# amolahinge/739-839-federated-learning-using-grpc

Measured on AMD Instinct MI355X. Metric: rounds/sec + samples/sec/client, 2-conv CNN FedAvg at 1/2/4/8 MI355X clients, higher is better.
Workload: dtype bf16; 1 GPU; model=lenet, global_batch=128, parallelism=fedavg-dp1, per_client_batch=128, local_epochs_per_round=1, eval_per_round=True, eval_split=full-per-client, data_split=strided-iid, aggregation=none (single client), hip_graph=True

## Files before the change

csrc/kernels/lenet_kernels.hip:

```cpp
#include <stdexcept>

#include "common.h"
#include "lenet_layout.h"

using namespace lenet;

#ifdef FEDMI_STAMPS
__device__ unsigned long long fedmi_stamps[FEDMI_STAMP_KERNELS][FEDMI_STAMP_WGS][FEDMI_STAMP_SLOTS];
__device__ int fedmi_ks1_diag;
#endif

namespace {

constexpr int NT_FWD = 512;
constexpr int NW_FWD = NT_FWD / 64;
constexpr int NT_CONV = 1024;
constexpr int NW_CONV = NT_CONV / 64;
constexpr int NT_FC = 512;

__constant__ float kMean[3] = {0.4914f, 0.4822f, 0.4465f};
__constant__ float kInvStd[3] = {1.f / 0.2023f, 1.f / 0.1994f, 1.f / 0.2010f};

FEDMI_DEV bf16x8 ld8(const bf16* p) { return *reinterpret_cast<const bf16x8*>(p); }

// ... 200 lines not shown
    const bf16* __restrict__ pk, const float* __restrict__ params, float* __restrict__ part)
{
  constexpr int SX_LD = F0P + 8;
  constexpr int XCH = F0P / 8;
  __shared__ __attribute__((aligned(16))) bf16 sX[16 * SX_LD];
  __shared__ __attribute__((aligned(16))) bf16 sH1[16 * 128];
  __shared__ __attribute__((aligned(16))) bf16 sH2[16 * 96];
  __shared__ float sZ[16 * 16];
  const int tid = threadIdx.x, lane = lane_id(), wave = wave_id();
  const int kq = (lane >> 4) * 8, n16 = lane & 15, rq = (lane >> 4) * 4;
  const int mt = blockIdx.x, s0 = mt * FC_SPW;
  const int ns = min(FC_SPW, nb - s0);
  if (ns <= 0) return;

  const int nf1 = wave * 16 + n16;
  bf16x8 w1f[13];
#pragma unroll
  for (int ks = 0; ks < 13; ++ks) w1f[ks] = ld8(pk + PK_FC1 + nf1 * F0P + ks * 32 + kq);
  const float b1 = params[P_F1B + min(nf1, F1 - 1)];
  const int nf2 = (wave < 6 ? wave : 0) * 16 + n16;
  const float b2 = params[P_F2B + min(nf2, F2 - 1)];
  const float b3 = params[P_F3B + min(n16, NCLS - 1)];
  bf16x8 w2f[4], w3f[3];
  if (wave < 6) {
#pragma unroll
    for (int ks = 0; ks < 4; ++ks) w2f[ks] = ld8(pk + PK_FC2 + nf2 * 128 + ks * 32 + kq);
  }
  if (wave == 0) {
#pragma unroll
    for (int ks = 0; ks < 3; ++ks) w3f[ks] = ld8(pk + PK_FC3 + n16 * 96 + ks * 32 + kq);
  }
  uint4 xv[2] = {make_uint4(0, 0, 0, 0), make_uint4(0, 0, 0, 0)};
#pragma unroll
  for (int u = 0; u < 2; ++u) {
    const int e = tid + u * NT_FC;
    if (e < 16 * XCH) {
      const int r = e / XCH;
      xv[u] = reinterpret_cast<const uint4*>(act2 + (size_t)(s0 + min(r, ns - 1)) * F0P)[e - r * XCH];
      if (r >= ns) xv[u] = make_uint4(0, 0, 0, 0);
    }
  }
#pragma unroll
  for (int u = 0; u < 2; ++u) {
    const int e = tid + u * NT_FC;
    if (e < 16 * XCH) {
      const int r = e / XCH;
      *reinterpret_cast<uint4*>(sX + r * SX_LD + (e - r * XCH) * 8) = xv[u];
    }
  }
  __syncthreads();

  {
    const bf16* xa = sX + n16 * SX_LD + kq;
    f32x4 acc = zero4();
#pragma unroll
    for (int ks = 0; ks < 13; ++ks) acc = mfma16(ld8(xa + ks * 32), w1f[ks], acc);
#pragma unroll
    for (int r = 0; r < 4; ++r) {
      const int sr = rq + r;
      sH1[sr * 128 + nf1] = (bf16)((nf1 < F1 && sr < ns) ? fmaxf(acc[r] + b1, 0.f) : 0.f);
    }
  }
  __syncthreads();
  if (wave < 6) {
    const bf16* ha = sH1 + n16 * 128 + kq;
    f32x4 acc = zero4();
#pragma unroll
    for (int ks = 0; ks < 4; ++ks) acc = mfma16(ld8(ha + ks * 32), w2f[ks], acc);
#pragma unroll
    for (int r = 0; r < 4; ++r) {
      const int sr = rq + r;
      sH2[sr * 96 + nf2] = (bf16)((nf2 < F2 && sr < ns) ? fmaxf(acc[r] + b2, 0.f) : 0.f);
    }
  }
  __syncthreads();
  if (wave == 0) {
    const bf16* ha = sH2 + n16 * 96 + kq;
    f32x4 acc = zero4();
#pragma unroll
    for (int ks = 0; ks < 3; ++ks) acc = mfma16(ld8(ha + ks * 32), w3f[ks], acc);
#pragma unroll
    for (int r = 0; r < 4; ++r) sZ[(rq + r) * 16 + n16] = acc[r] + b3;
  }
  __syncthreads();
  if (wave == 0) {
    float loss = 0.f, corr = 0.f;
    if (lane < ns) {
      float z[NCLS];
#pragma unroll
      for (int n = 0; n < NCLS; ++n) z[n] = sZ[lane * 16 + n];
      float mx = z[0]; int am = 0;
#pragma unroll
      for (int n = 1; n < NCLS; ++n) if (z[n] > mx) { mx = z[n]; am = n; }
      float se = 0.f;
#pragma unroll
      for (int n = 0; n < NCLS; ++n) se += __expf(z[n] - mx);
      const int y = labels[s0 + lane];
      float zy = 0.f;
#pragma unroll
      for (int n = 0; n < NCLS; ++n) zy = (n == y) ? z[n] : zy;
      loss = mx + __logf(se) - zy;
      corr = (am == y) ? 1.f : 0.f;
    }
    loss = wave_sum(loss);
    corr = wave_sum(corr);
    if (lane == 0) {
      part[2 * mt] = loss;
      part[2 * mt + 1] = corr;
    }
  }
}

constexpr int BW_XROW = 40, BW_XS_C = 32 * BW_XROW + 72, BW_XS_S = 3 * BW_XS_C + 48;
constexpr int BW_XSH = 5 * BW_XS_S;
constexpr int BW_P1SH = 5 * 6 * 14 * 16;
constexpr int BW_DY2W = 16 * 160;
constexpr int BW_DY2S = 24;
constexpr int BW_DY2C = 18 * 18 * BW_DY2S;
constexpr int BW_DY1S = 904;
constexpr int BW_DY1 = 6 * BW_DY1S;
constexpr int BW_WDGS = KDGP + 8;
constexpr int BW_O_XSH = 0, BW_O_P1SH = BW_O_XSH + BW_XSH * 2, BW_O_DY2W = BW_O_P1SH + BW_P1SH * 2,
              BW_O_DY2C = BW_O_DY2W + BW_DY2W * 2, BW_O_DY1 = BW_O_DY2C + BW_DY2C * 2,
              BW_O_DW1 = BW_O_DY1 + BW_DY1 * 2, BW_O_DB = BW_O_DW1 + 3 * 6 * 80 * 4, BW_SCRATCH = BW_O_DB + 64 * 4;

struct BwdLds {
  const uint8_t* raw;
  const bf16* p1r;
  const uint8_t* am1s;
  const uint8_t* am2s;
  const float* dxs;
  const bf16* wdg;
  bf16* xsh; bf16* p1sh; bf16* dY2w; bf16* dY2c; bf16* dY1; float* db; float* w1part;
};

FEDMI_DEV BwdLds bwd_lds(unsigned char* scratch, const uint8_t* raw, const bf16* p1r, const uint8_t* am1s,
                         const uint8_t* am2s, const float* dxs, const bf16* wdg) {
  BwdLds L;
  L.raw = raw; L.p1r = p1r; L.am1s = am1s; L.am2s = am2s; L.dxs = dxs; L.wdg = wdg;
  L.xsh = reinterpret_cast<bf16*>(scratch + BW_O_XSH);
  L.p1sh = reinterpret_cast<bf16*>(scratch + BW_O_P1SH);
  L.dY2w = reinterpret_cast<bf16*>(scratch + BW_O_DY2W);
  L.dY2c = reinterpret_cast<bf16*>(scratch + BW_O_DY2C);
  L.dY1 = reinterpret_cast<bf16*>(scratch + BW_O_DY1);
  L.w1part = reinterpret_cast<float*>(scratch + BW_O_DW1);
  L.db = reinterpret_cast<float*>(scratch + BW_O_DB);
  return L;
}

FEDMI_DEV void bwd_zero(const BwdLds& L) {
  zero_lds<NT_CONV>(L.dY2w, BW_DY2W * 2);
  zero_lds<NT_CONV>(L.dY2c, BW_DY2C * 2);
  zero_lds<NT_CONV>(L.dY1, BW_DY1 * 2);
  zero_lds<NT_CONV>(L.xsh, BW_XSH * 2);
  zero_lds<NT_CONV>(L.p1sh, BW_P1SH * 2);
  if (threadIdx.x < 64) L.db[threadIdx.x] = 0.f;
}

FEDMI_DEV void bwd_build_shifted_img(const BwdLds& L, const Aug& a, int tid, int nthr) {
  for (int e = tid; e < IMG_BYTES; e += nthr) {
    const int c = e >> 10, y = (e >> 5) & 31, x = e & 31;
    const bf16 v = (bf16)aug_pixel(L.raw, a, c, y, x);
    bf16* row = L.xsh + c * BW_XS_C + y * BW_XROW + x;
#pragma unroll
    for (int sh = 0; sh < 5; ++sh)
      if (x >= sh) row[sh * BW_XS_S - sh] = v;
  }
}
FEDMI_DEV void bwd_build_shifted_p1(const BwdLds& L, int tid, int nthr) {
  for (int e = tid; e < NP1; e += nthr) {
    const int c = e / 196, rem = e - c * 196, y = rem / P1, x = rem - y * P1;
    const bf16 v = L.p1r[e];
    bf16* row = L.p1sh + (c * 14 + y) * 16 + x;
#pragma unroll
    for (int sh = 0; sh < 5; ++sh)
      if (x >= sh) row[sh * (6 * 14 * 16) - sh] = v;
  }
}

FEDMI_DEV void bwd_main(const BwdLds& L, float* __restrict__ slab, int sk, int stamp_wg) {
  (void)sk; (void)stamp_wg;
  const int tid = threadIdx.x, lane = lane_id(), wave = wave_id();
  const int kq = (lane >> 4) * 8, n16 = lane & 15, rq = (lane >> 4) * 4;
  float* db = L.db;
  if (tid < C2 * 32) {
    const int o = tid >> 5, rem = tid & 31;
    float g = 0.f;
    if (rem < 25) {
      const int f = o * 25 + rem, py = rem / P2, px = rem - py * P2;
      const int am = L.am2s[f];
      const int y = 2 * py + (am >> 1), x = 2 * px + (am & 1);
      g = L.dxs[f];
      const bf16 gb = (bf16)g;
      L.dY2w[o * 160 + y * 16 + x] = gb;
      L.dY2c[((y + 4) * 18 + (x + 4)) * BW_DY2S + o] = gb;
    }
#pragma unroll
    for (int w = 1; w < 32; w <<= 1) g += __shfl_xor(g, w, 64);
    if (rem == 0) db[o] = g;
  }
  __syncthreads();
  FEDMI_STAMP(sk, 2);

  for (int t = wave - 7; t >= 0 && t < 10; t += 9) {
    const int kk = t * 16 + n16;
    const int kc = kk < 150 ? kk : 0;
    const int c = kc / 25, rs = kc - c * 25, r = rs / 5, sc = rs - r * 5;
    const bf16* bb = L.p1sh + ((sc * 6 + c) * 14 + r) * 16 + (kq & 15);
    f32x4 acc = zero4();
#pragma unroll
    for (int ks = 0; ks < 5; ++ks) {
      const int i = 2 * ks + (kq >> 4);
      acc = mfma16(ld8(L.dY2w + n16 * 160 + ks * 32 + kq), ld8(bb + i * 16), acc);
    }
    if (kk < 150) {
#pragma unroll
      for (int rr = 0; rr < 4; ++rr) slab[P_C2W + (rq + rr) * 150 + kk] = acc[rr];
    }
  }

  int koff[13];
#pragma unroll
  for (int ks = 0; ks < 13; ++ks) {
    const int G = ks * 4 + (lane >> 4), g = G >> 1;
    const int r = g / 5, sc = g - r * 5;
    koff[ks] = g < 25 ? (-r * 18 - sc) * BW_DY2S + (G & 1) * 8 : 0;
  }
  if (wave < 7) {
    const int ta = 2 * wave, tb = 2 * wave + 1;
    int pa = ta * 16 + n16, pb = tb * 16 + n16;
    if (pa >= 196) pa = 0;
    if (pb >= 196) pb = 0;
    const bf16* ga = L.dY2c + (((pa / P1) + 4) * 18 + (pa % P1 + 4)) * BW_DY2S;
    const bf16* gbb = L.dY2c + (((pb / P1) + 4) * 18 + (pb % P1 + 4)) * BW_DY2S;
    const bf16* wb = L.wdg + min(n16, C1) * BW_WDGS + kq;
    f32x4 acc[2] = {zero4(), zero4()};
#pragma unroll
    for (int ks = 0; ks < 13; ++ks) {
      const bf16x8 w = ld8(wb + ks * 32);
      acc[0] = mfma16(ld8(ga + koff[ks]), w, acc[0]);
      acc[1] = mfma16(ld8(gbb + koff[ks]), w, acc[1]);
    }
    FEDMI_STAMP(sk, 6);
    float csum = 0.f;
    if (n16 < C1) {
      const int c = n16;
#pragma unroll
      for (int h = 0; h < 2; ++h) {
        const int t = h ? tb : ta;
#pragma unroll
        for (int rr = 0; rr < 4; ++rr) {
          const int p = t * 16 + rq + rr;
          if (p < 196) {
            const int py = p / P1, px = p - py * P1;
            const float pooled = (float)L.p1r[c * 196 + p];
            const float g = pooled > 0.f ? acc[h][rr] : 0.f;
            const int am = L.am1s[c * 196 + p];
            const int yy = 2 * py + (am >> 1), xx = 2 * px + (am & 1);
            L.dY1[c * BW_DY1S + yy * 32 + xx] = (bf16)g;
            csum += g;
          }
        }
      }
    }
    csum += __shfl_xor(csum, 16, 64);
    csum += __shfl_xor(csum, 32, 64);
    if (n16 < C1 && lane < 16) db[16 + wave * C1 + n16] = csum;
    FEDMI_STAMP(sk, 7);
  }
  __syncthreads();
  FEDMI_STAMP(sk, 3);

  if (wave < 15) {
    const int nt = wave % 5, part = wave / 5;
    const int ks0 = part * 10, ks1 = min(ks0 + 10, O1);
    const int kk = nt * 16 + n16;
    const int kc = kk < 75 ? kk : kk - 64;
    const int c = kc / 25, rs = kc - c * 25, r = rs / 5, sc = rs - r * 5;
    const bf16* bb = L.xsh + sc * BW_XS_S + c * BW_XS_C + r * BW_XROW + kq;
    const bf16* ab = L.dY1 + min(n16, C1 - 1) * BW_DY1S + kq;
    const bool arow = n16 < C1;
    f32x4 acc0 = zero4(), acc1 = zero4();
    int ks = ks0;
    for (; ks + 1 < ks1; ks += 2) {
      bf16x8 a0 = ld8(ab + ks * 32), a1 = ld8(ab + ks * 32 + 32);
      if (!arow) { a0 = zero8(); a1 = zero8(); }
      acc0 = mfma16(a0, ld8(bb + ks * BW_XROW), acc0);
      acc1 = mfma16(a1, ld8(bb + (ks + 1) * BW_XROW), acc1);
    }
    if (ks < ks1) {
      bf16x8 a0 = ld8(ab + ks * 32);
      if (!arow) a0 = zero8();
      acc0 = mfma16(a0, ld8(bb + ks * BW_XROW), acc0);
    }
#pragma unroll
    for (int rr = 0; rr < 4; ++rr) {
      const int o = rq + rr;
      if (o < C1 && kk < 75) L.w1part[(part * 6 + o) * 80 + kk] = acc0[rr] + acc1[rr];
    }
  }
  __syncthreads();
  FEDMI_STAMP(sk, 4);
  for (int e = tid; e < C1 * 75; e += NT_CONV) {
    const int o = e / 75, kk = e - o * 75;
    slab[P_C1W + e] = L.w1part[o * 80 + kk] + L.w1part[(6 + o) * 80 + kk] + L.w1part[(12 + o) * 80 + kk];
  }
  if (tid < C1) {
    float b = 0.f;
#pragma unroll
    for (int w = 0; w < 7; ++w) b += db[16 + w * C1 + tid];
    slab[P_C1B + tid] = b;
  }
  if (tid < C2) slab[P_C2B + tid] = db[tid];
  FEDMI_STAMP(sk, 5);
}

constexpr int AUX_H2T = 0;
constexpr int AUX_DZ2T = AUX_H2T + 96 * 128 * 2;
constexpr int AUX_DZ3T = AUX_DZ2T + 96 * 128 * 2;
constexpr int FCB_N = 224;
constexpr int AUX_FCB = AUX_DZ3T + 16 * 128 * 2;
constexpr int AUX_LOSS = AUX_FCB + MAX_TRAIN_BATCH * FCB_N * 4;
constexpr int AUX_CORR = AUX_LOSS + MAX_TRAIN_BATCH * 4;
constexpr int AUX_BYTES = AUX_CORR + MAX_TRAIN_BATCH * 4;
static_assert(AUX_BYTES <= MAX_TRAIN_BATCH * F0 * 4, "FC side buffers must fit in dact2");

constexpr int S_O_RAW = 0, S_O_P1R = 3072, S_O_AM1 = S_O_P1R + 2368, S_O_AM2 = S_O_AM1 + 1184,
              S_O_X = S_O_AM2 + 416, S_O_DX = S_O_X + F0P * 2, S_O_WDG = S_O_DX + F0 * 4,
              S_O_FC = S_O_WDG + 16 * BW_WDGS * 2, S_O_W1C = S_O_FC + 2048, S_O_W2C = S_O_W1C + 16 * 136 * 2,
              S_O_SCR = S_O_W2C + 16 * 232 * 2;
constexpr int S_W1C_LD = 136, S_W2C_LD = 232;
constexpr int S_F_XCL = 0, S_F_C1 = S_F_XCL + 36 * 40 * 4 * 2, S_F_P1 = S_F_C1 + NPOS1 * 8 * 4,
              S_F_C2 = S_F_P1 + 14 * 14 * 8 * 2, S_F_END = S_F_C2 + C2 * NPOS2 * 4;
constexpr int S_O_RED = S_O_SCR + (S_F_END > BW_SCRATCH ? S_F_END : BW_SCRATCH);
constexpr int S_O_W3 = S_O_RED + NW_CONV * F0P * 4;
constexpr int S_END = S_O_W3 + 16 * 96 * 2;
static_assert(S_END <= 160 * 1024, "KS1 LDS");
constexpr int SF_H1 = 0, SF_H2 = 128, SF_Z = 224, SF_DZ3 = 240, SF_DZ2 = 256, SF_DZ1 = 352, SF_END = 480;
static_assert(SF_END * 4 <= 2048, "FC scratch");

FEDMI_DEV float dot8(const bf16x8& a, const bf16x8& b, float acc) {
#pragma unroll
  for (int j = 0; j < 8; ++j) acc += (float)a[j] * (float)b[j];
  return acc;
}
FEDMI_DEV float dot8f(const float* a, const bf16x8& b, float acc) {
#pragma unroll
  for (int j = 0; j < 8; ++j) acc += a[j] * (float)b[j];
  return acc;
}
FEDMI_DEV float sum8lanes(float v) {
  v += __shfl_xor(v, 1, 64);
  v += __shfl_xor(v, 2, 64);
  v += __shfl_xor(v, 4, 64);
  return v;
}
FEDMI_DEV float bfr(float v) { return (float)(bf16)v; }
FEDMI_DEV float row_sum16(float v) {
  v += __builtin_bit_cast(float, __builtin_amdgcn_mov_dpp(__builtin_bit_cast(int, v), 0x128, 0xf, 0xf, false));
  v += __builtin_bit_cast(float, __builtin_amdgcn_mov_dpp(__builtin_bit_cast(int, v), 0x124, 0xf, 0xf, false));
  v += __builtin_bit_cast(float, __builtin_amdgcn_mov_dpp(__builtin_bit_cast(int, v), 0x122, 0xf, 0xf, false));
  v += __builtin_bit_cast(float, __builtin_amdgcn_mov_dpp(__builtin_bit_cast(int, v), 0x121, 0xf, 0xf, false));
  return v;
}

__global__ __launch_bounds__(NT_CONV) void lenet_sample_step(
    const uint8_t* __restrict__ images, int sample_base, int nb,
    const bf16* __restrict__ pk, const float* __restrict__ params,
    uint32_t seed, const int* __restrict__ round_ctr, int augment,
    const int* __restrict__ labels,
    bf16* __restrict__ act2T,
    bf16* __restrict__ h1T,
    unsigned char* __restrict__ aux,
    bf16* __restrict__ dZ1T,
    float* __restrict__ conv_slab)
{
  __shared__ __attribute__((aligned(16))) unsigned char smem[S_END];
  const int s = blockIdx.x;
  if (s >= nb) return;
  [[maybe_unused]] const int stamp_wg = s;
  const int gidx = sample_base + s;
  const int tid = threadIdx.x, lane = lane_id(), wave = wave_id();
  const int kq = (lane >> 4) * 8, n16 = lane & 15, rq = (lane >> 4) * 4;
  uint8_t* raw = smem + S_O_RAW;
  bf16* p1r = reinterpret_cast<bf16*>(smem + S_O_P1R);
  uint8_t* am1s = smem + S_O_AM1;
  uint8_t* am2s = smem + S_O_AM2;
  bf16* xrow = reinterpret_cast<bf16*>(smem + S_O_X);
  float* dxs = reinterpret_cast<float*>(smem + S_O_DX);
  bf16* wdg = reinterpret_cast<bf16*>(smem + S_O_WDG);
  float* fcs = reinterpret_cast<float*>(smem + S_O_FC);
  float* red = reinterpret_cast<float*>(smem + S_O_RED);
  unsigned char* scr = smem + S_O_SCR;
  bf16* xcl = reinterpret_cast<bf16*>(scr + S_F_XCL);
  float* c1 = reinterpret_cast<float*>(scr + S_F_C1);
  bf16* p1cl = reinterpret_cast<bf16*>(scr + S_F_P1);
  float* c2 = reinterpret_cast<float*>(scr + S_F_C2);
  FEDMI_STAMP(0, 0);

  bf16* w1c = reinterpret_cast<bf16*>(smem + S_O_W1C);
  bf16* w2c = reinterpret_cast<bf16*>(smem + S_O_W2C);
  bf16* w3s = reinterpret_cast<bf16*>(smem + S_O_W3);
  float bias1, bias2;
  Aug a;
  {
    constexpr int NI = IMG_BYTES / 16, NWD = 16 * KDGP / 8, NW1 = 16 * K1C / 8, NW2 = 16 * K2C / 8, NW3 = 16 * 96 / 8;
    constexpr int E1 = NI, E2 = E1 + NWD, E3 = E2 + NW1, E4 = E3 + NW2, E5 = E4 + NW3;
    static_assert(E5 <= 2 * NT_CONV, "stage: two chunks per thread");
    uint4 v[2] = {make_uint4(0, 0, 0, 0), make_uint4(0, 0, 0, 0)};
#ifdef FEDMI_STAMPS
    const int dg = fedmi_ks1_diag;
    const size_t img_sample = (dg & 2) ? 0 : (size_t)gidx;
    const int lim = (dg & 1) ? E1 : E5;
#else
    const size_t img_sample = (size_t)gidx;
    constexpr int lim = E5;
#endif
#pragma unroll
    for (int u = 0; u < 2; ++u) {
      const int e = tid + u * NT_CONV;
      if (e < E1) v[u] = reinterpret_cast<const uint4*>(images + img_sample * IMG_BYTES)[e];
      else if (e >= lim) {}
      else if (e < E2) v[u] = reinterpret_cast<const uint4*>(pk + PK_W2DG)[e - E1];
      else if (e < E3) v[u] = reinterpret_cast<const uint4*>(pk + PK_W1C)[e - E2];
      else if (e < E4) v[u] = reinterpret_cast<const uint4*>(pk + PK_W2C)[e - E3];
      else if (e < E5) v[u] = reinterpret_cast<const uint4*>(pk + PK_FC3)[e - E4];
    }
    bias1 = n16 < C1 ? params[P_C1B + n16] : 0.f;
    bias2 = params[P_C2B + n16];
    a = aug_params(augment, seed, round_ctr, gidx);
    zero_lds<NT_CONV>(xcl, 36 * 40 * 4 * 2);
#pragma unroll
    for (int u = 0; u < 2; ++u) {
      const int e = tid + u * NT_CONV;
      if (e < E1) {
        reinterpret_cast<uint4*>(raw)[e] = v[u];
      } else if (e < E2) {
        const int w = e - E1, row = w / (KDGP / 8), col = w - row * (KDGP / 8);
        reinterpret_cast<uint4*>(wdg + row * BW_WDGS)[col] = v[u];
      } else if (e < E3) {
        const int w = e - E2, row = w / (K1C / 8), col = w - row * (K1C / 8);
        reinterpret_cast<uint4*>(w1c + row * S_W1C_LD)[col] = v[u];
      } else if (e < E4) {
        const int w = e - E3, row = w / (K2C / 8), col = w - row * (K2C / 8);
        reinterpret_cast<uint4*>(w2c + row * S_W2C_LD)[col] = v[u];
      } else if (e < E5) {
        reinterpret_cast<uint4*>(w3s)[e - E4] = v[u];
      }
    }
  }
  int go1[4], go2[7];
#pragma unroll
  for (int ks = 0; ks < 4; ++ks) {
    const int g = ks * 4 + (lane >> 4);
    go1[ks] = g < 15 ? ((g / 3) * 40 + 2 * (g % 3)) * 4 : 0;
  }
#pragma unroll
  for (int ks = 0; ks < 7; ++ks) {
    const int g = ks * 4 + (lane >> 4);
    go2[ks] = g < 25 ? ((g / 5) * P1 + (g % 5)) * 8 : 0;
  }
  __syncthreads();
  FEDMI_STAMP(1, 7);
  bf16x8 wb1[4];
#pragma unroll
  for (int ks = 0; ks < 4; ++ks) wb1[ks] = ld8(w1c + n16 * S_W1C_LD + ks * 32 + kq);
  for (int e = tid; e < IMG_BYTES; e += NT_CONV) {
    const int c = e >> 10, y = (e >> 5) & 31, x = e & 31;
    xcl[(y * 40 + x) * 4 + c] = (bf16)aug_pixel(raw, a, c, y, x);
  }
  __syncthreads();
  FEDMI_STAMP(0, 1);

  auto c1_row = [&](int tt) {
    const int q = tt * 4 + (n16 >> 2), y = 2 * (q / P1) + ((n16 >> 1) & 1), x = 2 * (q % P1) + (n16 & 1);
    return xcl + (y * 40 + x) * 4;
  };
  auto pool1 = [&](const f32x4& v, int tt) {
    if (n16 < 8) {
      const int q = tt * 4 + (lane >> 4);
      float m = fmaxf(v[0] + bias1, 0.f), c;
      int am = 0;
      c = fmaxf(v[1] + bias1, 0.f); if (c > m) { m = c; am = 1; }
      c = fmaxf(v[2] + bias1, 0.f); if (c > m) { m = c; am = 2; }
      c = fmaxf(v[3] + bias1, 0.f); if (c > m) { m = c; am = 3; }
      const bf16 mb = (bf16)m;
      p1cl[q * 8 + n16] = mb;
      if (n16 < C1) {
        p1r[n16 * 196 + q] = mb;
        am1s[n16 * 196 + q] = (uint8_t)am;
      }
    }
  };
  for (int t = wave; t < NPOS1 / 16; t += 2 * NW_CONV) {
    const int tb = t + NW_CONV;
    const bool two = tb < NPOS1 / 16;
    const bf16* xa = c1_row(t);
    const bf16* xbb = c1_row(two ? tb : t);
    bf16x8 fa[4], fb[4];
#pragma unroll
    for (int ks = 0; ks < 4; ++ks) {
      fa[ks] = ld8_b64x2(xa + go1[ks]);
      fb[ks] = ld8_b64x2(xbb + go1[ks]);
    }
    f32x4 acc = zero4(), accb = zero4();
#pragma unroll
    for (int ks = 0; ks < 4; ++ks) {
      acc = mfma16(fa[ks], wb1[ks], acc);
      accb = mfma16(fb[ks], wb1[ks], accb);
    }
    pool1(acc, t);
    if (two) pool1(accb, tb);
  }
  const int fn = tid >> 3, fq = tid & 7;
  constexpr int KCH = F0P / 8;
  const int kc = min(lane, KCH - 1);
  bf16x8 w1r[8];
#pragma unroll
  for (int m = 0; m < 8; ++m) w1r[m] = ld8(pk + PK_FC1 + (wave + 16 * m) * F0P + kc * 8);
  __syncthreads();
  FEDMI_STAMP(0, 2);
  FEDMI_STAMP(0, 3);

  if (wave < 7) {
    const int t = wave;
    int q = t * 4 + (n16 >> 2);
    if (q >= P2 * P2) q = 0;
    const int y = 2 * (q / P2) + ((n16 >> 1) & 1), x = 2 * (q % P2) + (n16 & 1);
    const bf16* pb = p1cl + (y * P1 + x) * 8;
    const bf16* wb = w2c + n16 * S_W2C_LD + kq;
    f32x4 acc = zero4();
#pragma unroll
    for (int ks = 0; ks < 7; ++ks) acc = mfma16(ld8(pb + go2[ks]), ld8(wb + ks * 32), acc);
    const int qo = t * 4 + (lane >> 4);
    if (qo < P2 * P2) {
      float m = fmaxf(acc[0] + bias2, 0.f), c;
      int am = 0;
      c = fmaxf(acc[1] + bias2, 0.f); if (c > m) { m = c; am = 1; }
      c = fmaxf(acc[2] + bias2, 0.f); if (c > m) { m = c; am = 2; }
      c = fmaxf(acc[3] + bias2, 0.f); if (c > m) { m = c; am = 3; }
      const bf16 mb = (bf16)m;
      const int e = n16 * (P2 * P2) + qo;
      am2s[e] = (uint8_t)am;
      xrow[e] = mb;
      act2T[(size_t)e * MAX_TRAIN_BATCH + s] = mb;
    }
  } else if (tid >= 7 * 64 && tid < 7 * 64 + (F0P - F0)) {
    const int e = F0 + tid - 7 * 64;
    xrow[e] = (bf16)0.f;
    act2T[(size_t)e * MAX_TRAIN_BATCH + s] = (bf16)0.f;
  }
  FEDMI_STAMP(0, 4);
  const int n2 = fn < 96 ? fn : 95;
  bf16x8 w2v[2];
#pragma unroll
  for (int i = 0; i < 2; ++i) w2v[i] = ld8(pk + PK_FC2 + n2 * 128 + fq * 8 + 64 * i);
  const int label = labels[s];
  const float fb1 = params[P_F1B + min(tid & 127, F1 - 1)];
  const float fb2 = params[P_F2B + min(fn, F2 - 1)];
  const float fb3 = params[P_F3B + min(fn, NCLS - 1)];
  __syncthreads();
  const BwdLds L = bwd_lds(scr, raw, p1r, am1s, am2s, dxs, wdg);
  bwd_zero(L);
  FEDMI_STAMP(0, 5);

  unsigned char* auxp = aux;
  float* fcb = reinterpret_cast<float*>(auxp + AUX_FCB) + (size_t)s * FCB_N;
  {
    const bf16x8 xv = ld8(xrow + kc * 8);
#pragma unroll
    for (int m = 0; m < 8; ++m) {
      const float p = row_sum16(lane < KCH ? dot8(xv, w1r[m], 0.f) : 0.f);
      if ((lane & 15) == 0) red[(wave + 16 * m) * 4 + (lane >> 4)] = p;
    }
  }
  bf16x8 w2t[2];
#pragma unroll
  for (int i = 0; i < 2; ++i) w2t[i] = ld8(pk + PK_FC2T + fn * 96 + min(fq * 8 + 64 * i, 88));
  __syncthreads();
  if (tid < 128) {
    const float* r = red + tid * 4;
    const float h = bfr(tid < F1 ? fmaxf(((r[0] + r[1]) + r[2]) + r[3] + fb1, 0.f) : 0.f);
    fcs[SF_H1 + tid] = h;
    h1T[(size_t)tid * MAX_TRAIN_BATCH + s] = (bf16)h;
  }
  __syncthreads();

  FEDMI_STAMP(1, 0);
  if (fn < 96) {
    float acc = 0.f;
#pragma unroll
    for (int i = 0; i < 2; ++i) acc = dot8f(fcs + SF_H1 + fq * 8 + 64 * i, w2v[i], acc);
    acc = sum8lanes(acc);
    if (fq == 0) {
      const float h = bfr(fn < F2 ? fmaxf(acc + fb2, 0.f) : 0.f);
      fcs[SF_H2 + fn] = h;
      reinterpret_cast<bf16*>(auxp + AUX_H2T)[(size_t)fn * MAX_TRAIN_BATCH + s] = (bf16)h;
    }
  }
  __syncthreads();
  FEDMI_STAMP(1, 1);
  if (fn < 16) {
    float acc = 0.f;
#pragma unroll
    for (int i = 0; i < 2; ++i)
      if (fq * 8 + 64 * i < 96) acc = dot8f(fcs + SF_H2 + fq * 8 + 64 * i, ld8(w3s + fn * 96 + fq * 8 + 64 * i), acc);
    acc = sum8lanes(acc);
    if (fq == 0) fcs[SF_Z + fn] = fn < NCLS ? acc + fb3 : 0.f;
  } else {
    bwd_build_shifted_img(L, a, tid - 128, NT_CONV - 128);
  }
  __syncthreads();
  FEDMI_STAMP(1, 2);
  if (wave == 0) {
    const int n = lane & 15;
    const float zn = n < NCLS ? fcs[SF_Z + n] : -INFINITY;
    float mx = zn;
#pragma unroll
    for (int o = 1; o < 16; o <<= 1) mx = fmaxf(mx, __shfl_xor(mx, o, 64));
    float cand = (zn == mx) ? (float)n : 16.f;
#pragma unroll
    for (int o = 1; o < 16; o <<= 1) cand = fminf(cand, __shfl_xor(cand, o, 64));
    float se = n < NCLS ? __expf(zn - mx) : 0.f;
#pragma unroll
    for (int o = 1; o < 16; o <<= 1) se += __shfl_xor(se, o, 64);
    const float lse = mx + __logf(se);
    const int y = label;
    const float zy = __shfl(zn, y, 64);
    const float d = n < NCLS ? (__expf(zn - lse) - (n == y ? 1.f : 0.f)) * (1.f / (float)nb) : 0.f;
    if (lane < 16) {
      fcs[SF_DZ3 + n] = bfr(d);
      reinterpret_cast<bf16*>(auxp + AUX_DZ3T)[(size_t)n * MAX_TRAIN_BATCH + s] = (bf16)d;
      if (n < NCLS) fcb[204 + n] = d;
    }
    if (lane == 0) {
      reinterpret_cast<float*>(auxp + AUX_LOSS)[s] = lse - zy;
      reinterpret_cast<float*>(auxp + AUX_CORR)[s] = ((int)cand == y) ? 1.f : 0.f;
    }
  } else {
    bwd_build_shifted_p1(L, tid - 64, NT_CONV - 64);
  }
  __syncthreads();
  FEDMI_STAMP(1, 3);
  if (tid < 96) {
    float acc = 0.f;
#pragma unroll
    for (int n = 0; n < NCLS; ++n) acc += fcs[SF_DZ3 + n] * (float)w3s[n * 96 + tid];
    const float g = (tid < F2 && fcs[SF_H2 + tid] > 0.f) ? acc : 0.f;
    fcs[SF_DZ2 + tid] = bfr(g);
    reinterpret_cast<bf16*>(auxp + AUX_DZ2T)[(size_t)tid * MAX_TRAIN_BATCH + s] = (bf16)g;
    if (tid < F2) fcb[120 + tid] = g;
  }
  __syncthreads();
  FEDMI_STAMP(1, 4);
  {
    float acc = 0.f;
#pragma unroll
    for (int i = 0; i < 2; ++i)
      if (fq * 8 + 64 * i < 96) acc = dot8f(fcs + SF_DZ2 + fq * 8 + 64 * i, w2t[i], acc);
    acc = sum8lanes(acc);
    if (fq == 0) {
      const float g = (fn < F1 && fcs[SF_H1 + fn] > 0.f) ? acc : 0.f;
      fcs[SF_DZ1 + fn] = bfr(g);
      dZ1T[(size_t)fn * DZ1_LD + s] = (bf16)g;
      if (fn < F1) fcb[fn] = g;
    }
  }
  __syncthreads();
  FEDMI_STAMP(1, 5);
  {
    float d[8];
#pragma unroll
    for (int j = 0; j < 8; ++j) d[j] = 0.f;
#pragma unroll
    for (int m = 0; m < 8; ++m) {
      const float g = fcs[SF_DZ1 + wave + 16 * m];
#pragma unroll
      for (int j = 0; j < 8; ++j) d[j] += g * (float)w1r[m][j];
    }
    if (lane < KCH) {
      float4* o = reinterpret_cast<float4*>(red + wave * F0P + lane * 8);
      o[0] = make_float4(d[0], d[1], d[2], d[3]);
      o[1] = make_float4(d[4], d[5], d[6], d[7]);
    }
  }
  __syncthreads();
  if (tid < F0) {
    float acc = 0.f;
#pragma unroll
    for (int w = 0; w < NW_CONV; ++w) acc += red[w * F0P + tid];
    dxs[tid] = (float)xrow[tid] > 0.f ? acc : 0.f;
  }
  __syncthreads();
  FEDMI_STAMP(0, 6);
  bwd_main(L, conv_slab + (size_t)s * CS, 2, stamp_wg);
}

FEDMI_DEV void pack_one(int i, float w, bf16* __restrict__ pk) {
  const bf16 v = (bf16)w;
  if (i < P_C1B) {
    const int o = i / 75, k = i - o * 75, c = k / 25, rs = k - c * 25, r = rs / 5, s = rs - r * 5;
    pk[PK_W1C + o * K1C + (r * 3 + (s >> 1)) * 8 + (s & 1) * 4 + c] = v;
  } else if (i < P_C2W) {
  } else if (i < P_C2B) {
    const int j = i - P_C2W, o = j / 150, k = j - o * 150, c = k / 25, rs = k - c * 25;
    pk[PK_W2C + o * K2C + rs * 8 + c] = v;
    pk[PK_W2DG + c * KDGP + rs * 16 + o] = v;
  } else if (i < P_F1W) {
  } else if (i < P_F1B) {
    const int j = i - P_F1W, n = j / F0, f = j - n * F0;
    pk[PK_FC1 + n * F0P + f] = v;
  } else if (i < P_F2W) {
  } else if (i < P_F2B) {
    const int j = i - P_F2W, n = j / F1, f = j - n * F1;
    pk[PK_FC2 + n * 128 + f] = v;
    pk[PK_FC2T + f * 96 + n] = v;
  } else if (i < P_F3W) {
  } else if (i < P_F3B) {
    const int j = i - P_F3W, n = j / F2, f = j - n * F2;
    pk[PK_FC3 + n * 96 + f] = v;
  }
}

__global__ __launch_bounds__(256) void lenet_pack(const float* __restrict__ params, bf16* __restrict__ pk) {
  const int i = blockIdx.x * 256 + threadIdx.x;
  if (i < P_TOTAL) pack_one(i, params[i], pk);
}

constexpr int SGD_NA = (CS + 15) / 16;

FEDMI_DEV void sgd_apply(int i, float grad, float p, float m, float* __restrict__ params, float* __restrict__ mom,
                         bf16* __restrict__ pk, float lr, float momentum, float wd) {
  const float d = grad + wd * p;
  const float b = momentum * m + d;
  const float np = p - lr * b;
  mom[i] = b;
  params[i] = np;
  pack_one(i, np, pk);
}

FEDMI_DEV bf16x8 mask_cols(bf16x8 v, int s0, int nb) {
  if (s0 + 8 <= nb) return v;
#pragma unroll
  for (int j = 0; j < 8; ++j)
    if (s0 + j >= nb) v[j] = (bf16)0.f;
  return v;
}

FEDMI_DEV f32x4 batch_tile(const bf16* __restrict__ a, const bf16* __restrict__ b, int nb,
                           const float* __restrict__ params, const float* __restrict__ mom, const int* idx,
                           float* p, float* m) {
  const int lane = lane_id(), kq = (lane >> 4) * 8, n16 = lane & 15;
  bf16x8 av[4], bv[4];
#pragma unroll
  for (int ks = 0; ks < 4; ++ks) {
    av[ks] = ld8(a + n16 * MAX_TRAIN_BATCH + ks * 32 + kq);
    bv[ks] = ld8(b + n16 * MAX_TRAIN_BATCH + ks * 32 + kq);
  }
#pragma unroll
  for (int r = 0; r < 4; ++r) {
    p[r] = params[idx[r] >= 0 ? idx[r] : 0];
    m[r] = mom[idx[r] >= 0 ? idx[r] : 0];
  }
  f32x4 acc = zero4();
#pragma unroll
  for (int ks = 0; ks < 4; ++ks)
    acc = mfma16(mask_cols(av[ks], ks * 32 + kq, nb), mask_cols(bv[ks], ks * 32 + kq, nb), acc);
  return acc;
}

constexpr int SGD2_NB = (8 * 25 + 3) / 4;
constexpr int SGD2_NC = (6 * 8 + 3) / 4;
constexpr int SGD2_ND = (6 + 3) / 4;
constexpr int SGD2_NE = 4;
constexpr int SGD2_GRID = SGD_NA + SGD2_NB + SGD2_NC + SGD2_ND + SGD2_NE + 1;

__global__ __launch_bounds__(256) void lenet_sgd2(
    float* __restrict__ params, float* __restrict__ mom, bf16* __restrict__ pk,
    const float* __restrict__ conv_slab, int nb,
    const bf16* __restrict__ act2T, const bf16* __restrict__ h1T, const unsigned char* __restrict__ aux,
    const bf16* __restrict__ dZ1T, float lr, float momentum, float wd,
    int* __restrict__ round_ctr, Stats* __restrict__ stats)
{
  __shared__ float red[16][17];
  const int b = blockIdx.x, tid = threadIdx.x, wave = wave_id(), lane = lane_id();
  const int n16 = lane & 15, rq = (lane >> 4) * 4;
  [[maybe_unused]] const int stamp_wg = b;
  FEDMI_STAMP(3, 0);
  if (b < SGD_NA) {
    const int pl = tid & 15, g = tid >> 4;
    const int i = b * 16 + pl;
    float p = 0.f, m = 0.f;
    if (g == 0 && i < CS) { p = params[i]; m = mom[i]; }
    float sum = 0.f;
    if (i < CS) {
      float v[MAX_TRAIN_BATCH / 16];
#pragma unroll
      for (int u = 0; u < MAX_TRAIN_BATCH / 16; ++u) v[u] = conv_slab[(size_t)min(g + 16 * u, nb - 1) * CS + i];
#pragma unroll
      for (int u = 0; u < MAX_TRAIN_BATCH / 16; ++u) sum += g + 16 * u < nb ? v[u] : 0.f;
    }
    red[g][pl] = sum;
    __syncthreads();
    if (g == 0 && i < CS) {
      float tot = 0.f;
#pragma unroll
      for (int q = 0; q < 16; ++q) tot += red[q][pl];
      sgd_apply(i, tot, p, m, params, mom, pk, lr, momentum, wd);
    }
  } else if (b < SGD_NA + SGD2_NB) {
    const int t = (b - SGD_NA) * 4 + wave;
    if (t < 200) {
      const int nt = t / 25, ft = t - nt * 25;
      int idx[4];
      float p[4], m[4];
#pragma unroll
      for (int r = 0; r < 4; ++r) {
        const int n = nt * 16 + rq + r, f = ft * 16 + n16;
        idx[r] = n < F1 ? P_F1W + n * F0 + f : -1;
      }
      const f32x4 acc = batch_tile(dZ1T + (size_t)nt * 16 * DZ1_LD, act2T + (size_t)ft * 16 * MAX_TRAIN_BATCH, nb,
                                   params, mom, idx, p, m);
      FEDMI_STAMP(3, 2);
#pragma unroll
      for (int r = 0; r < 4; ++r)
        if (idx[r] >= 0) sgd_apply(idx[r], acc[r], p[r], m[r], params, mom, pk, lr, momentum, wd);
      FEDMI_STAMP(3, 3);
    }
  } else if (b < SGD_NA + SGD2_NB + SGD2_NC) {
    const int t = (b - SGD_NA - SGD2_NB) * 4 + wave;
    if (t < 48) {
      const int nt = t >> 3, ft = t & 7;
      const bf16* dz2t = reinterpret_cast<const bf16*>(aux + AUX_DZ2T);
      int idx[4];
      float p[4], m[4];
#pragma unroll
      for (int r = 0; r < 4; ++r) {
        const int n = nt * 16 + rq + r, f = ft * 16 + n16;
        idx[r] = (n < F2 && f < F1) ? P_F2W + n * F1 + f : -1;
      }
      const f32x4 acc = batch_tile(dz2t + (size_t)nt * 16 * MAX_TRAIN_BATCH, h1T + (size_t)ft * 16 * MAX_TRAIN_BATCH, nb,
                                   params, mom, idx, p, m);
#pragma unroll
      for (int r = 0; r < 4; ++r)
        if (idx[r] >= 0) sgd_apply(idx[r], acc[r], p[r], m[r], params, mom, pk, lr, momentum, wd);
    }
  } else if (b < SGD_NA + SGD2_NB + SGD2_NC + SGD2_ND) {
    const int t = (b - SGD_NA - SGD2_NB - SGD2_NC) * 4 + wave;
    if (t < 6) {
      const bf16* dz3t = reinterpret_cast<const bf16*>(aux + AUX_DZ3T);
      const bf16* h2t = reinterpret_cast<const bf16*>(aux + AUX_H2T);
      int idx[4];
      float p[4], m[4];
#pragma unroll
      for (int r = 0; r < 4; ++r) {
        const int n = rq + r, f = t * 16 + n16;
        idx[r] = (n < NCLS && f < F2) ? P_F3W + n * F2 + f : -1;
      }
      const f32x4 acc = batch_tile(dz3t, h2t + (size_t)t * 16 * MAX_TRAIN_BATCH, nb, params, mom, idx, p, m);
#pragma unroll
      for (int r = 0; r < 4; ++r)
        if (idx[r] >= 0) sgd_apply(idx[r], acc[r], p[r], m[r], params, mom, pk, lr, momentum, wd);
    }
  } else {
    const int e = b - (SGD_NA + SGD2_NB + SGD2_NC + SGD2_ND);
    const float* fcb = reinterpret_cast<const float*>(aux + AUX_FCB);
    const int j = e * 64 + (tid & 63), g = tid >> 6;
    __shared__ float bsum[4][64];
    float bp = 0.f, bm = 0.f;
    const int bi = j < 120 ? P_F1B + j : (j < 204 ? P_F2B + j - 120 : P_F3B + j - 204);
    if (e < SGD2_NE && g == 0 && j < 214) { bp = params[bi]; bm = mom[bi]; }
    if (e < SGD2_NE && j < 214) {
      float v[32];
#pragma unroll
      for (int u = 0; u < 32; ++u) v[u] = fcb[(size_t)min(g * 32 + u, nb - 1) * FCB_N + j];
      float sum = 0.f;
#pragma unroll
      for (int u = 0; u < 32; ++u) sum += g * 32 + u < nb ? v[u] : 0.f;
      bsum[g][tid & 63] = sum;
    } else if (e == SGD2_NE && g == 0 && stats != nullptr) {
      const float* lv = reinterpret_cast<const float*>(aux + AUX_LOSS);
      const float* cv = reinterpret_cast<const float*>(aux + AUX_CORR);
      float ls = 0.f, cs = 0.f;
#pragma unroll
      for (int u = 0; u < 2; ++u) {
        const int sm = lane + 64 * u;
        if (sm < nb) { ls += lv[sm]; cs += cv[sm]; }
      }
      ls = wave_sum(ls);
      cs = wave_sum(cs);
      if (lane == 0) {
        stats->loss_sum += ls;
        stats->correct += (int)(cs + 0.5f);
        stats->count += nb;
      }
    }
    __syncthreads();
    if (e < SGD2_NE && g == 0 && j < 214) {
      const float sum = (bsum[0][tid] + bsum[1][tid]) + (bsum[2][tid] + bsum[3][tid]);
      sgd_apply(bi, sum, bp, bm, params, mom, pk, lr, momentum, wd);
    }
  }
  if (b == 0 && tid == 0 && round_ctr) atomicAdd(round_ctr, 1);
  FEDMI_STAMP(3, 1);
}

namespace fedmi {

void launch_lenet_conv_fwd(hipStream_t st, const uint8_t* images, int sample_base, int nb,
                           const bf16* pk, const float* params, uint32_t seed, const int* round_ctr,
                           int augment, bf16* act2, bf16* act2T, int tstride, bf16* pool1,
                           uint8_t* am1, uint8_t* am2, Stats* zero_stats) {
  if (nb <= 0) return;
  hipLaunchKernelGGL(lenet_conv_fwd, dim3(nb), dim3(NT_FWD), 0, st, images, sample_base, nb, pk, params,
                     seed, round_ctr, augment, act2, act2T, tstride, pool1, am1, am2, zero_stats);
}

__global__ __launch_bounds__(256) void lenet_eval_stats(const float* __restrict__ part, int groups, int n,
                                                        Stats* __restrict__ stats) {
  __shared__ float rl[256], rc[256];
// ... 84 lines not shown
```

Baseline: 5.481 million samples/s.

## Overlap backward shifted-tile builds with forward conv and trim LDS work

Result: faster. 5.672 million samples/s (median of 6 runs) (+3.5%).

```diff
diff --git a/csrc/kernels/lenet_kernels.hip b/csrc/kernels/lenet_kernels.hip
--- a/csrc/kernels/lenet_kernels.hip
+++ b/csrc/kernels/lenet_kernels.hip
@@ -376,35 +376,56 @@
   zero_lds<NT_CONV>(L.dY2w, BW_DY2W * 2);
   zero_lds<NT_CONV>(L.dY2c, BW_DY2C * 2);
   zero_lds<NT_CONV>(L.dY1, BW_DY1 * 2);
-  zero_lds<NT_CONV>(L.xsh, BW_XSH * 2);
-  zero_lds<NT_CONV>(L.p1sh, BW_P1SH * 2);
-  if (threadIdx.x < 64) L.db[threadIdx.x] = 0.f;
-}
-
-FEDMI_DEV void bwd_build_shifted_img(const BwdLds& L, const Aug& a, int tid, int nthr) {
-  for (int e = tid; e < IMG_BYTES; e += nthr) {
-    const int c = e >> 10, y = (e >> 5) & 31, x = e & 31;
-    const bf16 v = (bf16)aug_pixel(L.raw, a, c, y, x);
-    bf16* row = L.xsh + c * BW_XS_C + y * BW_XROW + x;
-#pragma unroll
-    for (int sh = 0; sh < 5; ++sh)
-      if (x >= sh) row[sh * BW_XS_S - sh] = v;
+  const int tid = threadIdx.x;
+  if (tid < 512) {
+    const int sh = 1 + (tid >> 7), c = (tid >> 5) & 3, y = tid & 31;
+    if (c < 3) *reinterpret_cast<uint2*>(L.xsh + sh * BW_XS_S + c * BW_XS_C + y * BW_XROW + 28) = make_uint2(0, 0);
+  } else if (tid < 512 + BW_P1SH / 16) {
+    *reinterpret_cast<uint4*>(L.p1sh + (tid - 512) * 16 + 8) = make_uint4(0, 0, 0, 0);
+  }
+  if (tid < 64) L.db[tid] = 0.f;
+}
+static_assert((BW_XS_S * 2) % 8 == 0 && (BW_XS_C * 2) % 8 == 0 && (BW_XROW * 2) % 8 == 0 && BW_O_P1SH % 16 == 0,
+              "tail clears are aligned 8 / 16-byte stores");
+static_assert(512 + BW_P1SH / 16 <= NT_CONV, "one tail clear per thread");
+
+FEDMI_DEV void store_shifted_pairs(bf16* row, int copy_stride, int x, unsigned p01, unsigned p12) {
+#pragma unroll
+  for (int sh = 0; sh < 5; ++sh) {
+    if (sh & 1) {
+      if (x + 1 >= sh) *reinterpret_cast<unsigned*>(row + sh * copy_stride + 1 - sh) = p12;
+    } else {
+      if (x >= sh) *reinterpret_cast<unsigned*>(row + sh * copy_stride - sh) = p01;
+    }
+  }
+}
+FEDMI_DEV unsigned pack2(bf16 lo, bf16 hi) {
+  return (unsigned)__builtin_bit_cast(unsigned short, lo) | ((unsigned)__builtin_bit_cast(unsigned short, hi) << 16);
+}
+FEDMI_DEV void bwd_build_shifted_img(const BwdLds& L, const bf16* xcl, int tid, int nthr) {
+  for (int e = tid; e < 3 * IMG * (IMG / 2); e += nthr) {
+    const int c = e >> 9, y = (e >> 4) & 31, x = 2 * (e & 15);
+    const bf16* px = xcl + (y * 40 + x) * 4 + c;
+    const bf16 v0 = px[0], v1 = px[4], v2 = px[8];
+    store_shifted_pairs(L.xsh + c * BW_XS_C + y * BW_XROW + x, BW_XS_S, x, pack2(v0, v1), pack2(v1, v2));
   }
 }
 FEDMI_DEV void bwd_build_shifted_p1(const BwdLds& L, int tid, int nthr) {
-  for (int e = tid; e < NP1; e += nthr) {
-    const int c = e / 196, rem = e - c * 196, y = rem / P1, x = rem - y * P1;
-    const bf16 v = L.p1r[e];
-    bf16* row = L.p1sh + (c * 14 + y) * 16 + x;
-#pragma unroll
-    for (int sh = 0; sh < 5; ++sh)
-      if (x >= sh) row[sh * (6 * 14 * 16) - sh] = v;
-  }
-}
+  for (int e = tid; e < C1 * P1 * 8; e += nthr) {
+    const int rw = e >> 3, x = 2 * (e & 7);
+    if (x >= P1) continue;
+    const bf16* pv = L.p1r + rw * P1 + x;
+    const bf16 v0 = pv[0], v1 = pv[1], v2 = x + 2 < P1 ? pv[2] : (bf16)0.f;
+    store_shifted_pairs(L.p1sh + rw * 16 + x, 6 * 14 * 16, x, pack2(v0, v1), pack2(v1, v2));
+  }
+}
+static_assert(BW_XS_S % 2 == 0 && BW_XS_C % 2 == 0 && BW_XROW % 2 == 0 && BW_O_P1SH % 4 == 0, "pair stores are 4-byte aligned");
 
 FEDMI_DEV void bwd_main(const BwdLds& L, float* __restrict__ slab, int sk, int stamp_wg) {
   (void)sk; (void)stamp_wg;
-  const int tid = threadIdx.x, lane = lane_id(), wave = wave_id();
+  int lane = lane_id();
+  asm volatile("" : "+v"(lane));
+  const int tid = threadIdx.x, wave = wave_id();
   const int kq = (lane >> 4) * 8, n16 = lane & 15, rq = (lane >> 4) * 4;
   float* db = L.db;
   if (tid < C2 * 32) {
@@ -443,14 +464,14 @@
     }
   }
 
-  int koff[13];
-#pragma unroll
-  for (int ks = 0; ks < 13; ++ks) {
-    const int G = ks * 4 + (lane >> 4), g = G >> 1;
-    const int r = g / 5, sc = g - r * 5;
-    koff[ks] = g < 25 ? (-r * 18 - sc) * BW_DY2S + (G & 1) * 8 : 0;
-  }
   if (wave < 7) {
+    int koff[13];
+#pragma unroll
+    for (int ks = 0; ks < 13; ++ks) {
+      const int G = ks * 4 + (lane >> 4), g = G >> 1;
+      const int r = g / 5, sc = g - r * 5;
+      koff[ks] = g < 25 ? (-r * 18 - sc) * BW_DY2S + (G & 1) * 8 : 0;
+    }
     const int ta = 2 * wave, tb = 2 * wave + 1;
     int pa = ta * 16 + n16, pb = tb * 16 + n16;
     if (pa >= 196) pa = 0;
@@ -472,14 +493,18 @@
 #pragma unroll
       for (int h = 0; h < 2; ++h) {
         const int t = h ? tb : ta;
-#pragma unroll
-        for (int rr = 0; rr < 4; ++rr) {
-          const int p = t * 16 + rq + rr;
-          if (p < 196) {
-            const int py = p / P1, px = p - py * P1;
-            const float pooled = (float)L.p1r[c * 196 + p];
+        const int p0 = t * 16 + rq;
+        if (p0 < 196) {
+          const int py0 = p0 / P1, px0 = p0 - py0 * P1;
+          const uint2 pv = *reinterpret_cast<const uint2*>(L.p1r + c * 196 + p0);
+          const unsigned av = *reinterpret_cast<const unsigned*>(L.am1s + c * 196 + p0);
+#pragma unroll
+          for (int rr = 0; rr < 4; ++rr) {
+            const int wrap = px0 + rr >= P1, py = py0 + wrap, px = px0 + rr - wrap * P1;
+            const unsigned w = rr < 2 ? pv.x : pv.y;
+            const float pooled = __builtin_bit_cast(float, (rr & 1) ? (w & 0xffff0000u) : (w << 16));
             const float g = pooled > 0.f ? acc[h][rr] : 0.f;
-            const int am = L.am1s[c * 196 + p];
+            const int am = (av >> (8 * rr)) & 3;
             const int yy = 2 * py + (am >> 1), xx = 2 * px + (am & 1);
             L.dY1[c * BW_DY1S + yy * 32 + xx] = (bf16)g;
             csum += g;
@@ -525,9 +550,10 @@
   }
   __syncthreads();
   FEDMI_STAMP(sk, 4);
-  for (int e = tid; e < C1 * 75; e += NT_CONV) {
-    const int o = e / 75, kk = e - o * 75;
-    slab[P_C1W + e] = L.w1part[o * 80 + kk] + L.w1part[(6 + o) * 80 + kk] + L.w1part[(12 + o) * 80 + kk];
+  if (tid < C1 * 128) {
+    const int o = tid >> 7, kk = tid & 127;
+    if (kk < 75)
+      slab[P_C1W + o * 75 + kk] = L.w1part[o * 80 + kk] + L.w1part[(6 + o) * 80 + kk] + L.w1part[(12 + o) * 80 + kk];
   }
   if (tid < C1) {
     float b = 0.f;
@@ -554,12 +580,13 @@
               S_O_FC = S_O_WDG + 16 * BW_WDGS * 2, S_O_W1C = S_O_FC + 2048, S_O_W2C = S_O_W1C + 16 * 136 * 2,
               S_O_SCR = S_O_W2C + 16 * 232 * 2;
 constexpr int S_W1C_LD = 136, S_W2C_LD = 232;
-constexpr int S_F_XCL = 0, S_F_C1 = S_F_XCL + 36 * 40 * 4 * 2, S_F_P1 = S_F_C1 + NPOS1 * 8 * 4,
-              S_F_C2 = S_F_P1 + 14 * 14 * 8 * 2, S_F_END = S_F_C2 + C2 * NPOS2 * 4;
-constexpr int S_O_RED = S_O_SCR + (S_F_END > BW_SCRATCH ? S_F_END : BW_SCRATCH);
+constexpr int S_O_RED = S_O_SCR + BW_SCRATCH;
+constexpr int S_R_XCL = 128 * 4 * 4, S_R_P1 = S_R_XCL + 36 * 40 * 4 * 2, S_R_END = S_R_P1 + 14 * 14 * 8 * 2;
+static_assert(S_R_END <= NW_CONV * F0P * 4 && S_O_RED % 16 == 0, "forward images fit behind the fc1 partials");
 constexpr int S_O_W3 = S_O_RED + NW_CONV * F0P * 4;
 constexpr int S_END = S_O_W3 + 16 * 96 * 2;
 static_assert(S_END <= 160 * 1024, "KS1 LDS");
+static_assert(S_O_P1R % 8 == 0 && S_O_AM1 % 4 == 0, "pool1 backward reads 4 positions per access");
 constexpr int SF_H1 = 0, SF_H2 = 128, SF_Z = 224, SF_DZ3 = 240, SF_DZ2 = 256, SF_DZ1 = 352, SF_END = 480;
 static_assert(SF_END * 4 <= 2048, "FC scratch");
 
@@ -615,11 +642,9 @@
   bf16* wdg = reinterpret_cast<bf16*>(smem + S_O_WDG);
   float* fcs = reinterpret_cast<float*>(smem + S_O_FC);
   float* red = reinterpret_cast<float*>(smem + S_O_RED);
-  unsigned char* scr = smem + S_O_SCR;
-  bf16* xcl = reinterpret_cast<bf16*>(scr + S_F_XCL);
-  float* c1 = reinterpret_cast<float*>(scr + S_F_C1);
-  bf16* p1cl = reinterpret_cast<bf16*>(scr + S_F_P1);
-  float* c2 = reinterpret_cast<float*>(scr + S_F_C2);
+  bf16* xcl = reinterpret_cast<bf16*>(smem + S_O_RED + S_R_XCL);
+  bf16* p1cl = reinterpret_cast<bf16*>(smem + S_O_RED + S_R_P1);
+  const BwdLds L = bwd_lds(smem + S_O_SCR, raw, p1r, am1s, am2s, dxs, wdg);
   FEDMI_STAMP(0, 0);
 
   bf16* w1c = reinterpret_cast<bf16*>(smem + S_O_W1C);
@@ -654,6 +679,7 @@
     bias2 = params[P_C2B + n16];
     a = aug_params(augment, seed, round_ctr, gidx);
     zero_lds<NT_CONV>(xcl, 36 * 40 * 4 * 2);
+    bwd_zero(L);
 #pragma unroll
     for (int u = 0; u < 2; ++u) {
       const int e = tid + u * NT_CONV;
@@ -673,16 +699,11 @@
       }
     }
   }
-  int go1[4], go2[7];
+  int go1[4];
 #pragma unroll
   for (int ks = 0; ks < 4; ++ks) {
     const int g = ks * 4 + (lane >> 4);
     go1[ks] = g < 15 ? ((g / 3) * 40 + 2 * (g % 3)) * 4 : 0;
-  }
-#pragma unroll
-  for (int ks = 0; ks < 7; ++ks) {
-    const int g = ks * 4 + (lane >> 4);
-    go2[ks] = g < 25 ? ((g / 5) * P1 + (g % 5)) * 8 : 0;
   }
   __syncthreads();
   FEDMI_STAMP(1, 7);
@@ -753,6 +774,12 @@
     const int y = 2 * (q / P2) + ((n16 >> 1) & 1), x = 2 * (q % P2) + (n16 & 1);
     const bf16* pb = p1cl + (y * P1 + x) * 8;
     const bf16* wb = w2c + n16 * S_W2C_LD + kq;
+    int go2[7];
+#pragma unroll
+    for (int ks = 0; ks < 7; ++ks) {
+      const int g = ks * 4 + (lane >> 4);
+      go2[ks] = g < 25 ? ((g / 5) * P1 + (g % 5)) * 8 : 0;
+    }
     f32x4 acc = zero4();
 #pragma unroll
     for (int ks = 0; ks < 7; ++ks) acc = mfma16(ld8(pb + go2[ks]), ld8(wb + ks * 32), acc);
@@ -769,10 +796,14 @@
       xrow[e] = mb;
       act2T[(size_t)e * MAX_TRAIN_BATCH + s] = mb;
     }
-  } else if (tid >= 7 * 64 && tid < 7 * 64 + (F0P - F0)) {
-    const int e = F0 + tid - 7 * 64;
-    xrow[e] = (bf16)0.f;
-    act2T[(size_t)e * MAX_TRAIN_BATCH + s] = (bf16)0.f;
+    bwd_build_shifted_p1(L, tid, 7 * 64);
+  } else {
+    if (tid < 7 * 64 + (F0P - F0)) {
+      const int e = F0 + tid - 7 * 64;
+      xrow[e] = (bf16)0.f;
+      act2T[(size_t)e * MAX_TRAIN_BATCH + s] = (bf16)0.f;
+    }
+    bwd_build_shifted_img(L, xcl, tid - 7 * 64, NT_CONV - 7 * 64);
   }
   FEDMI_STAMP(0, 4);
   const int n2 = fn < 96 ? fn : 95;
@@ -784,8 +815,6 @@
   const float fb2 = params[P_F2B + min(fn, F2 - 1)];
   const float fb3 = params[P_F3B + min(fn, NCLS - 1)];
   __syncthreads();
-  const BwdLds L = bwd_lds(scr, raw, p1r, am1s, am2s, dxs, wdg);
-  bwd_zero(L);
   FEDMI_STAMP(0, 5);
 
   unsigned char* auxp = aux;
@@ -831,13 +860,13 @@
       if (fq * 8 + 64 * i < 96) acc = dot8f(fcs + SF_H2 + fq * 8 + 64 * i, ld8(w3s + fn * 96 + fq * 8 + 64 * i), acc);
     acc = sum8lanes(acc);
     if (fq == 0) fcs[SF_Z + fn] = fn < NCLS ? acc + fb3 : 0.f;
-  } else {
-    bwd_build_shifted_img(L, a, tid - 128, NT_CONV - 128);
   }
   __syncthreads();
   FEDMI_STAMP(1, 2);
   if (wave == 0) {
-    const int n = lane & 15;
+    int ln = lane;
+    asm volatile("" : "+v"(ln));
+    const int n = ln & 15;
     const float zn = n < NCLS ? fcs[SF_Z + n] : -INFINITY;
     float mx = zn;
 #pragma unroll
@@ -861,8 +890,6 @@
       reinterpret_cast<float*>(auxp + AUX_LOSS)[s] = lse - zy;
       reinterpret_cast<float*>(auxp + AUX_CORR)[s] = ((int)cand == y) ? 1.f : 0.f;
     }
-  } else {
-    bwd_build_shifted_p1(L, tid - 64, NT_CONV - 64);
   }
   __syncthreads();
   FEDMI_STAMP(1, 3);
@@ -987,9 +1014,14 @@
     m[r] = mom[idx[r] >= 0 ? idx[r] : 0];
   }
   f32x4 acc = zero4();
-#pragma unroll
-  for (int ks = 0; ks < 4; ++ks)
-    acc = mfma16(mask_cols(av[ks], ks * 32 + kq, nb), mask_cols(bv[ks], ks * 32 + kq, nb), acc);
+  if (nb == MAX_TRAIN_BATCH) {
+#pragma unroll
+    for (int ks = 0; ks < 4; ++ks) acc = mfma16(av[ks], bv[ks], acc);
+  } else {
+#pragma unroll
+    for (int ks = 0; ks < 4; ++ks)
+      acc = mfma16(mask_cols(av[ks], ks * 32 + kq, nb), mask_cols(bv[ks], ks * 32 + kq, nb), acc);
+  }
   return acc;
 }
 
```
